# ruiguo-bio/smer_music_generation

Hardware: AMD Instinct MI355X
Metric: infill tokens/sec + train tokens/sec, SMER seq_len=1024, 1/2/4/8 MI355X (higher is better)
Workload: dtype bf16; 1 GPU; C2 train step: 6+6 layers d512 h8 ff2048 V309, per-GPU B=32 S=1024 T=256, dropout 0.1, fused WCE + Adam; global_batch=32, seq_len=1024, tgt_len=256, parallelism=dp1

## Files before the change

### include/smer_hip.h

```cpp
#ifndef SMER_HIP_H
#define SMER_HIP_H

#include <stddef.h>
#include <stdint.h>

#ifdef __cplusplus
extern "C" {
#endif

typedef struct ihipStream_t* smer_stream_t;

#define SMER_OK 0
#define SMER_ERR_INVALID (-1)
#define SMER_ERR_HIP (-2)
#define SMER_ERR_UNSUPPORTED (-3)

#define SMER_F32 0
#define SMER_BF16 1

int smer_abi_version(void);
const char* smer_last_error(void);

int smer_gemm(int dtype, int a_kcontig, int b_kcontig, int M, int N, int K,
              const void* A, long lda, const void* B, long ldb,
// ... 196 lines not shown
                         smer_stream_t stream);
int smer_bar_clock(int R, int V, float* logits, long ldl, const int32_t* state, int nst,
                   const int8_t* targets, int max_masks, const int32_t* out_tok, int cap,
                   const uint8_t* cls, const uint8_t* units, int eos, const int32_t* bar_len,
                   int32_t* clock, smer_stream_t stream);

int smer_layernorm_fwd(int dtype, int M, int N, const void* x, long ldx,
                       const float* gamma, const float* beta, float eps,
                       void* y, long ldy, float* mean, float* rstd, smer_stream_t stream);
size_t smer_layernorm_bwd_workspace(int M, int N);
int smer_layernorm_bwd(int dtype, int M, int N, const void* dy, long lddy, int dy_f32,
                       const void* x, long ldx, const float* mean, const float* rstd,
                       const float* gamma, void* dx, long lddx,
                       void* dx_drop, long ldxd, float drop_p, uint32_t seed,
                       float* dgamma, float* dbeta, int accumulate,
                       void* workspace, size_t ws_bytes, smer_stream_t stream);
int smer_layernorm_bwd_partials(int dtype, int M, int N, const void* dy, long lddy, int dy_f32,
                                const void* x, long ldx, const float* mean, const float* rstd,
                                const float* gamma, void* dx, long lddx, void* dx_drop,
                                long ldxd, float drop_p, uint32_t seed, void* workspace,
                                size_t ws_bytes, smer_stream_t stream);
int smer_layernorm_param_reduce(int M, int N, void* workspace, size_t ws_bytes, float* dgamma,
                                float* dbeta, int accumulate, smer_stream_t stream);

int smer_embed_fwd(int dtype, int n_tok, int d, const int64_t* ids, const int32_t* positions,
                   int L, const float* table, const float* pe, float scale,
                   float drop_p, uint32_t seed, void* out, long ldo, smer_stream_t stream);
int smer_embed_fwd_fp8(int n_tok, int d, const int64_t* ids, const int32_t* positions, int L,
                       const float* table, const float* pe, float scale, float drop_p, uint32_t seed,
                       void* out, long ldo, void* q8, long ldq, const float* qs, unsigned* amax,
                       smer_stream_t stream);
size_t smer_embed_bwd_workspace(int V, int d, int n_tok_total);
int smer_embed_bwd(int dtype, int V, int d, float scale,
                   const int64_t* ids0, const void* dx0, long ld0, int n0, float p0, uint32_t seed0,
                   const int64_t* ids1, const void* dx1, long ld1, int n1, float p1, uint32_t seed1,
                   float* dtable, void* workspace, size_t ws_bytes, smer_stream_t stream);

int smer_wce_denom(int n, const int64_t* y, const float* ce_all, float* denom,
                   smer_stream_t stream);
int smer_wce_fwd_bwd(int dtype, int R, int V, const float* logits, long ldl, const int64_t* y,
                     const float* w, const float* denom, float* row_loss, float* loss_out,
                     void* dlogits, long ldd, float grad_scale, smer_stream_t stream);

int smer_adam(long n, float* p, const float* g, float* m, float* v, void* p_bf16,
              float lr, float b1, float b2, float eps, float bc1, float bc2_sqrt,
              smer_stream_t stream);
// ... 59 lines not shown
```

### smer_music_generation_amd/_lib.py

```python
from __future__ import annotations

import ctypes
import os

import torch

_HERE = os.path.dirname(os.path.abspath(__file__))
LIB_PATH = os.environ.get("SMER_HIP_LIB") or os.path.join(_HERE, "libsmer_hip.so")

c_int, c_long, c_float, c_size, c_u32 = (ctypes.c_int, ctypes.c_long, ctypes.c_float,
                                         ctypes.c_size_t, ctypes.c_uint32)
P = ctypes.c_void_p

SIGNATURES = {
    "smer_abi_version": (c_int, []),
    "smer_last_error": (ctypes.c_char_p, []),
    "smer_gemm": (c_int, [c_int, c_int, c_int, c_int, c_int, c_int, P, c_long, P, c_long, P,
                          c_float, c_int, P, c_long, P, c_long, c_float, c_float, c_u32, P,
                          c_long, P, c_long, c_int, P, c_size, P]),
    "smer_gemm_debug_stamps": (c_int, [P, c_size]),
    "smer_gemm_plan": (c_int, [c_int, c_int, c_int, c_int, c_int, c_int, ctypes.c_uint, c_long, c_size, c_int,
                               c_int, P]),
    "smer_gemm_kernel_name": (ctypes.c_char_p, [c_int]),
    "smer_attn_fwd_plan": (c_int, [c_int, c_int, c_int, c_int, c_int, c_int, ctypes.c_uint, P]),
# ... 81 lines not shown
    "smer_grammar_sample_step": (c_int, [c_int, c_int, P, c_long, P, c_int, P, c_int, P, P, P,
                                         c_int, c_int, c_int, c_int, P, P, P, P, c_int, P, P, P,
                                         c_int, P]),
    "smer_grammar_sample_step_tp": (c_int, [c_int, c_int, P, c_long, P, c_int, P, c_int, P, P, P,
                                            c_int, c_int, c_int, c_int, P, P, P, P, c_int, P, P, P,
                                            c_int, P, P]),
    "smer_grammar_sample_step_rows": (c_int, [c_int, c_int, P, c_long, P, c_int, P, c_int, P, P, P,
                                              c_int, c_int, c_int, c_int, P, P, P, P, c_int, P, c_long,
                                              P, P, c_int, P, P]),
    "smer_logits_ban": (c_int, [c_int, c_int, P, c_long, P, c_int, c_int, P, P, c_int, P]),
    "smer_logprob_stage": (c_int, [c_int, c_int, P, c_long, P, c_int, P, c_int, P, P, c_long, P, P]),
    "smer_logprob_commit": (c_int, [c_int, c_int, P, c_int, P, P, c_int, P, c_long, P, P]),
    "smer_logprob_rows": (c_int, [c_int, c_int, c_int, P, c_long, P, P, P, P, P, c_int, P, P, P, P]),
    "smer_logits_template": (c_int, [c_int, c_int, P, c_long, P, c_int, P, P, c_int, c_int, P]),
    "smer_bar_clock": (c_int, [c_int, c_int, P, c_long, P, c_int, P, c_int, P, c_int, P, P, c_int, P, P, P]),
    "smer_layernorm_fwd": (c_int, [c_int, c_int, c_int, P, c_long, P, P, c_float, P, c_long, P,
                                   P, P]),
    "smer_layernorm_bwd_workspace": (c_size, [c_int, c_int]),
    "smer_layernorm_bwd": (c_int, [c_int, c_int, c_int, P, c_long, c_int, P, c_long, P, P, P, P,
                                   c_long, P, c_long, c_float, c_u32, P, P, c_int, P, c_size, P]),
    "smer_layernorm_bwd_partials": (c_int, [c_int, c_int, c_int, P, c_long, c_int, P, c_long, P, P,
                                            P, P, c_long, P, c_long, c_float, c_u32, P, c_size, P]),
    "smer_layernorm_param_reduce": (c_int, [c_int, c_int, P, c_size, P, P, c_int, P]),
    "smer_embed_fwd": (c_int, [c_int, c_int, c_int, P, P, c_int, P, P, c_float, c_float, c_u32,
                               P, c_long, P]),
    "smer_embed_bwd_workspace": (c_size, [c_int, c_int, c_int]),
    "smer_embed_bwd": (c_int, [c_int, c_int, c_int, c_float, P, P, c_long, c_int, c_float, c_u32,
                               P, P, c_long, c_int, c_float, c_u32, P, P, c_size, P]),
    "smer_wce_denom": (c_int, [c_int, P, P, P, P]),
    "smer_wce_fwd_bwd": (c_int, [c_int, c_int, c_int, P, c_long, P, P, P, P, P, P, c_long,
                                 c_float, P]),
    "smer_adam": (c_int, [c_long, P, P, P, P, P, c_float, c_float, c_float, c_float, c_float,
                          c_float, P]),
    "smer_cast": (c_int, [c_int, c_int, c_long, P, P, P]),
    "smer_cast2d": (c_int, [c_int, c_int, c_int, c_int, P, c_long, P, c_long, P]),
    "smer_colsum_workspace": (c_size, [c_int, c_int]),
    "smer_colsum": (c_int, [c_int, c_int, c_int, P, c_long, P, c_int, P, c_size, P]),
    "smer_debug_checksum": (c_int, [P, c_long, c_long, c_long, P, c_int, P]),
    "smer_argmax_accuracy": (c_int, [c_int, c_int, P, c_long, P, P, c_int, c_int, P, P]),
}

_lib = None
_load_error = None


def load():
# ... 29 lines not shown
```

### smer_music_generation_amd/csrc/common.h

```cpp
#pragma once
#include <hip/hip_runtime.h>
#include <stdint.h>

#include "../../include/smer_hip.h"

typedef __bf16 bf16;
typedef __bf16 bf16x8 __attribute__((ext_vector_type(8)));
typedef __bf16 bf16x4 __attribute__((ext_vector_type(4)));
typedef short i16x4 __attribute__((ext_vector_type(4)));
typedef float f32x4 __attribute__((ext_vector_type(4)));

#define SMER_WAVE 64

extern "C" int smer_set_error(int code, const char* msg);
#define SMER_CHECK_LAUNCH(what)                                          \
  do {                                                                   \
    hipError_t _e = hipGetLastError();                                   \
    if (_e != hipSuccess) return smer_set_error(SMER_ERR_HIP, hipGetErrorString(_e)); \
  } while (0)
#define SMER_REQUIRE(cond, msg) \
  do { if (!(cond)) return smer_set_error(SMER_ERR_INVALID, msg); } while (0)

template <typename T> __device__ __forceinline__ float to_f32(T x);
template <> __device__ __forceinline__ float to_f32<float>(float x) { return x; }
// ... 70 lines not shown
  h = __umul24(h, 0x6CA68Bu);
  h ^= h >> 16;
  return h;
}
__device__ __forceinline__ uint32_t smer_attn_ge(uint32_t h, uint32_t lo4) {
  return (h | 0x80808080u) - lo4;
}
__device__ __forceinline__ bool smer_attn_keep(uint32_t rowkey, uint32_t thr7, uint32_t key) {
  return ((smer_attn_bits(rowkey, key >> 2) >> (8 * (key & 3))) & 0x7Fu) >= thr7;
}
static inline uint32_t smer_attn_thr7(float p) {
  if (p <= 0.f) return 0u;
  long t = (long)((double)p * 128.0 + 0.5);
  return (uint32_t)(t < 1 ? 1 : (t > 127 ? 127 : t));
}
static inline float smer_attn_scale7(uint32_t thr7) {
  return thr7 ? (float)(128.0 / (128.0 - (double)thr7)) : 1.f;
}

size_t smer_col_reduce_scratch(int nblk, int N);
void smer_col_reduce_launch(int nblk, int N, const float* part, long stride, long off, float* out,
                            int accumulate, float scale, float* scratch, hipStream_t s,
                            float* out2 = nullptr, int nsplit = 0);

template <typename T, bool VEC = true>
__device__ __forceinline__ void load8(const T* p, int valid, float (&v)[8]) {
  if (VEC && valid >= 8) {
    if constexpr (sizeof(T) == 2) {
      bf16x8 r = *reinterpret_cast<const bf16x8*>(p);
#pragma unroll
      for (int i = 0; i < 8; ++i) v[i] = (float)r[i];
    } else {
      float4 a = *reinterpret_cast<const float4*>(p), b = *reinterpret_cast<const float4*>(p + 4);
      v[0] = a.x; v[1] = a.y; v[2] = a.z; v[3] = a.w; v[4] = b.x; v[5] = b.y; v[6] = b.z; v[7] = b.w;
    }
  } else {
#pragma unroll
    for (int i = 0; i < 8; ++i) v[i] = i < valid ? (float)p[i] : 0.f;
  }
}

constexpr int LNR_MAXC = 4;
template <int NC = LNR_MAXC>
__device__ __forceinline__ void ln_stats_loaded(const float (&v)[NC][8], int N, float eps, int lane, float& mu,
                                                float& rs) {
  const int nch = N >> 3;
// ... 168 lines not shown
```

### smer_music_generation_amd/csrc/norm_embed.hip

```cpp
#include "common.h"

namespace {
constexpr int LN_MAXC = 4;

template <typename T> struct Vec8;
template <> struct Vec8<bf16> {
  static __device__ __forceinline__ void load(const bf16* p, float (&v)[8]) {
    bf16x8 r = *reinterpret_cast<const bf16x8*>(p);
#pragma unroll
    for (int i = 0; i < 8; ++i) v[i] = (float)r[i];
  }
  static __device__ __forceinline__ void store(bf16* p, const float (&v)[8]) {
    bf16x8 r;
#pragma unroll
    for (int i = 0; i < 8; ++i) r[i] = (bf16)v[i];
    *reinterpret_cast<bf16x8*>(p) = r;
  }
};
template <> struct Vec8<float> {
  static __device__ __forceinline__ void load(const float* p, float (&v)[8]) {
    float4 a = *reinterpret_cast<const float4*>(p), b = *reinterpret_cast<const float4*>(p + 4);
    v[0] = a.x; v[1] = a.y; v[2] = a.z; v[3] = a.w; v[4] = b.x; v[5] = b.y; v[6] = b.z; v[7] = b.w;
  }
  static __device__ __forceinline__ void store(float* p, const float (&v)[8]) {
// ... 735 lines not shown
  if (!occ[which]) {
    int nb = 0;
    const void* kern = which == 2   ? (const void*)ln_bwd_t4_kernel<4>
                       : which == 0 ? (const void*)ln_bwd_kernel<bf16, false, 2, 2, true>
                                    : (const void*)ln_bwd_kernel<bf16, false, 4, 1, true>;
    if (hipOccupancyMaxActiveBlocksPerMultiprocessor(&nb, kern, 256, 0) != hipSuccess || nb <= 0) nb = 1;
    occ[which] = nb;
  }
  int dev = 0, cus = 256;
  if (hipGetDevice(&dev) != hipSuccess ||
      hipDeviceGetAttribute(&cus, hipDeviceAttributeMultiprocessorCount, dev) != hipSuccess || cus <= 0)
    cus = 256;
  const long resident = (long)cus * occ[which];
  const long per = (M + resident - 1) / resident;
  const int rows = (int)((per + 15) / 16 * 16);
  return rows > fixed ? fixed : rows;
}

extern "C" size_t smer_layernorm_bwd_workspace(int M, int N) {
  size_t nblk = (size_t)(M + ln_bwd_rows(M, N) - 1) / ln_bwd_rows(M, N);
  return nblk * 2 * N * sizeof(float) + smer_col_reduce_scratch((int)nblk, 2 * N);
}

static int ln_bwd_impl(int dtype, int M, int N, const void* dy, long lddy, int dy_f32,
                       const void* x, long ldx, const float* mean, const float* rstd,
                       const float* gamma, void* dx, long lddx, void* dx_drop, long ldxd,
                       float drop_p, uint32_t seed, float* dgamma, float* dbeta, int accumulate,
                       void* workspace, size_t ws_bytes, smer_stream_t stream, bool params,
                       bool reduce, uint8_t* q8 = nullptr, long ldq = 0, const float* qs = nullptr,
                       unsigned* amax = nullptr) {
  SMER_REQUIRE(N % 8 == 0 && N <= 64 * 8 * LN_MAXC, "smer_layernorm_bwd: N % 8 == 0 and N <= 2048");
  SMER_REQUIRE(dx && dy && x && mean && rstd && gamma, "smer_layernorm_bwd: null pointer");
  SMER_REQUIRE(!params || (workspace && ws_bytes >= smer_layernorm_bwd_workspace(M, N)),
               "smer_layernorm_bwd: workspace too small");
  if (M == 0) return SMER_OK;
  hipStream_t s = (hipStream_t)stream;
  const int rpb = ln_bwd_rows(M, N);
  int nblk = (M + rpb - 1) / rpb;
  uint32_t thr = smer_drop_thr16(drop_p);
  float ds = smer_drop_scale16(thr);
  float* part = params ? (float*)workspace : nullptr;
  SMER_REQUIRE(((uintptr_t)gamma & 15) == 0, "smer_layernorm_bwd: gamma must be 16-B aligned");
#define LNB2(T, F, NC, RB, PF)                                                                 \
  hipLaunchKernelGGL((ln_bwd_kernel<T, F, NC, RB, PF>), dim3(nblk), dim3(256), 0, s, M, N, dy, \
                     lddy, (const T*)x, ldx, mean, rstd, gamma, (T*)dx, lddx, (T*)dx_drop, ldxd, \
                     thr, seed, ds, part, rpb)
#define LNB1(T, F, NC, RB)                                          \
  do {                                                              \
    if (rpb / 4 > (RB)) LNB2(T, F, NC, RB, true);                   \
    else LNB2(T, F, NC, RB, false);                                 \
  } while (0)
#define LNB(T, F)                                  \
  do {                                             \
    if (N <= 512) LNB1(T, F, 1, 4);                \
    else if (N <= 1024) LNB1(T, F, 2, 2);          \
    else LNB1(T, F, 4, 1);                         \
// ... 99 lines not shown

extern "C" int smer_layernorm_param_reduce(int M, int N, void* workspace, size_t ws_bytes,
                                           float* dgamma, float* dbeta, int accumulate,
                                           smer_stream_t stream) {
  SMER_REQUIRE(workspace && ws_bytes >= smer_layernorm_bwd_workspace(M, N),
               "smer_layernorm_param_reduce: workspace too small");
  if (M == 0 || (!dgamma && !dbeta)) return SMER_OK;
  const int nblk = (M + ln_bwd_rows(M, N) - 1) / ln_bwd_rows(M, N);
  float* part = (float*)workspace;
  hipStream_t s = (hipStream_t)stream;
  if (dgamma && dbeta)
    smer_col_reduce_launch(nblk, 2 * N, part, (long)2 * N, 0L, dgamma, accumulate, 1.f,
                           part + (size_t)nblk * 2 * N, s, dbeta, N);
  else if (dgamma)
    smer_col_reduce_launch(nblk, N, part, (long)2 * N, 0L, dgamma, accumulate, 1.f,
                           part + (size_t)nblk * 2 * N, s);
  else
    smer_col_reduce_launch(nblk, N, part, (long)2 * N, (long)N, dbeta, accumulate, 1.f,
                           part + (size_t)nblk * 2 * N, s);
  SMER_CHECK_LAUNCH("smer_layernorm_param_reduce");
  return SMER_OK;
}

extern "C" int smer_embed_fwd(int dtype, int n_tok, int d, const int64_t* ids,
                              const int32_t* positions, int L, const float* table,
                              const float* pe, float scale, float drop_p, uint32_t seed,
                              void* out, long ldo, smer_stream_t stream) {
  SMER_REQUIRE(d % 4 == 0, "smer_embed_fwd: d % 4 == 0");
  SMER_REQUIRE(positions || L > 0, "smer_embed_fwd: L");
  if (n_tok == 0) return SMER_OK;
  hipStream_t s = (hipStream_t)stream;
  long tot = (long)n_tok * (d / 4);
  uint32_t thr = smer_drop_thr16(drop_p);
  float ds = smer_drop_scale16(thr);
  if (dtype == SMER_BF16)
    hipLaunchKernelGGL(embed_fwd_kernel<bf16>, dim3((tot + 255) / 256), dim3(256), 0, s, n_tok, d,
                       ids, positions, L, table, pe, scale, thr, seed, ds, (bf16*)out, ldo);
  else if (dtype == SMER_F32)
    hipLaunchKernelGGL(embed_fwd_kernel<float>, dim3((tot + 255) / 256), dim3(256), 0, s, n_tok, d,
                       ids, positions, L, table, pe, scale, thr, seed, ds, (float*)out, ldo);
  else
    return smer_set_error(SMER_ERR_UNSUPPORTED, "smer_embed_fwd: dtype");
  SMER_CHECK_LAUNCH("smer_embed_fwd");
  return SMER_OK;
}

// ... 59 lines not shown
```

### smer_music_generation_amd/csrc/train_ops.hip

```cpp
#include "common.h"

__global__ __launch_bounds__(256) void wce_denom_kernel(int n, const int64_t* __restrict__ y,
                                                        const float* __restrict__ ce_all,
                                                        float* __restrict__ denom) {
  __shared__ float red[256];
  float a = 0.f;
  for (int i = threadIdx.x; i < n; i += 256) a += ce_all[y[i]];
  red[threadIdx.x] = a;
  __syncthreads();
  for (int s = 128; s > 0; s >>= 1) {
    if (threadIdx.x < s) red[threadIdx.x] += red[threadIdx.x + s];
    __syncthreads();
  }
  if (threadIdx.x == 0) *denom = red[0];
}

template <typename T>
__global__ __launch_bounds__(256) void wce_kernel(int R, int V, const float* __restrict__ logits,
                                                  long ldl, const int64_t* __restrict__ y,
                                                  const float* __restrict__ w,
                                                  const float* __restrict__ denom,
                                                  float* __restrict__ row_loss,
                                                  T* __restrict__ dlog, long ldd,
                                                  float grad_scale) {
// ... 133 lines not shown

size_t smer_col_reduce_scratch(int nblk, int N) {
  return nblk > 64 ? (size_t)((nblk + 63) / 64) * N * sizeof(float) : 0;
}

void smer_col_reduce_launch(int nblk, int N, const float* part, long stride, long off, float* out,
                            int accumulate, float scale, float* scratch, hipStream_t s,
                            float* out2, int nsplit) {
  dim3 gx((N + 63) / 64);
  if (!out2) nsplit = N;
  if (nblk > 64) {
    int g = (nblk + 63) / 64;
    hipLaunchKernelGGL(smer_col_reduce, dim3(gx.x, g), dim3(256), 0, s, nblk, N, part, stride,
                       off, scratch, (long)N, 64, 0, 1.f, (float*)nullptr, N);
    hipLaunchKernelGGL(smer_col_reduce, dim3(gx.x, 1), dim3(256), 0, s, g, N,
                       (const float*)scratch, (long)N, 0L, out, 0L, g, accumulate, scale, out2,
                       nsplit);
  } else {
    hipLaunchKernelGGL(smer_col_reduce, dim3(gx.x, 1), dim3(256), 0, s, nblk, N, part, stride,
                       off, out, 0L, nblk, accumulate, scale, out2, nsplit);
  }
}

extern "C" int smer_wce_denom(int n, const int64_t* y, const float* ce_all, float* denom,
                              smer_stream_t stream) {
  SMER_REQUIRE(y && ce_all && denom, "smer_wce_denom: null pointer");
  hipLaunchKernelGGL(wce_denom_kernel, dim3(1), dim3(256), 0, (hipStream_t)stream, n, y, ce_all,
                     denom);
  SMER_CHECK_LAUNCH("smer_wce_denom");
  return SMER_OK;
}

extern "C" int smer_wce_fwd_bwd(int dtype, int R, int V, const float* logits, long ldl,
                                const int64_t* y, const float* w, const float* denom,
                                float* row_loss, float* loss_out, void* dlogits, long ldd,
                                float grad_scale, smer_stream_t stream) {
  SMER_REQUIRE(logits && y && w && denom && row_loss, "smer_wce_fwd_bwd: null pointer");
  if (R == 0) return SMER_OK;
  hipStream_t s = (hipStream_t)stream;
  dim3 grid((R + 3) / 4);
  if (dtype == SMER_BF16)
    hipLaunchKernelGGL(wce_kernel<bf16>, grid, dim3(256), 0, s, R, V, logits, ldl, y, w, denom,
                       row_loss, (bf16*)dlogits, ldd, grad_scale);
  else if (dtype == SMER_F32)
    hipLaunchKernelGGL(wce_kernel<float>, grid, dim3(256), 0, s, R, V, logits, ldl, y, w, denom,
                       row_loss, (float*)dlogits, ldd, grad_scale);
// ... 184 lines not shown
```

### smer_music_generation_amd/engine.py

```python
from __future__ import annotations

import math
import os

import torch

from . import ops

_SITE = {"pe_src": 1, "pe_tgt": 2}


def _site(kind, layer, which):
    return 16 + (layer * 16 + which) * 2 + (0 if kind == "enc" else 1)


class _W:
    pass


FP8_FFN2 = os.environ.get("SMER_FP8_FFN2", "1") == "1"
FP8_EMBED = os.environ.get("SMER_FP8_EMBED", "0") == "1"
FP8_H8 = (os.environ.get("SMER_FP8_H8", "1") == "1"
          and os.environ.get("SMER_FP8_Q8_FAST", "1") != "0")


_WGRAD_SIDE_CAP = int(os.environ.get("SMER_WGRAD_SIDE_CAP", "0"))
_WGRAD_FP8_CAP = int(os.environ.get("SMER_WGRAD_FP8_CAP", "192"))
_ATTN_MASK_PREGEN = os.environ.get("SMER_ATTN_MASK_PREGEN", "0") == "1"


class Engine:
    def __init__(self, model):
        self.m = model
        self.d = model.d_model
        self.H = model.nhead
        self.D = self.d // self.H
        self.F = model.dim_feedforward
        self.V = model.vocab_size
        self.Vp = (self.V + 63) // 64 * 64
        self.n_enc = model.num_encoder_layers
        self.n_dec = model.num_decoder_layers
        self._bf16 = None
        self._bf16_version = None
        self._fc_pad = None
        self._wgen = 0
        self._ckv_all = None
        self._side = {}
        self._mstream = {}
        self._fp8 = None

    def act_dtype(self):
        return torch.float32 if self.m.precision == "fp32" else torch.bfloat16

    def _weights_flat(self, dt):
        flat = self.m.flat_parameters()
        if dt == torch.float32:
            return flat
        ver = self._version_key()
        if self._bf16 is None or self._bf16.numel() != flat.numel() or self._bf16_version != ver:
            if self._bf16 is None or self._bf16.numel() != flat.numel():
                self._bf16 = torch.empty(flat.numel(), dtype=torch.bfloat16, device=flat.device)
            ops.cast(flat, self._bf16)
            self._fc_pad = None
            self._bf16_version = ver
            self._wgen += 1
        return self._bf16

    def _version_key(self):
        flat = self.m.flat_parameters()
        return (flat.data_ptr(), flat._version, sum(p._version for p in self.m.parameters()))

    def mark_bf16_fresh(self):
# ... 365 lines not shown
                return
            if x is None or dy is None:
                raise RuntimeError("engine: fp8 weight gradient declined with no bf16 input")
            ops.linear_wgrad(dy, x, gw, ws=ws, max_wg=cap, **kw)
        if side is None:
            run(None, 0)
            return
        stream, ws = side
        stream.wait_stream(torch.cuda.current_stream(side[1].device))
        with torch.cuda.stream(stream):
            run(ws, _WGRAD_SIDE_CAP)
            if ops.CK_LOG is not None:
                ops.ck("S:dW", gw)
                ops.ck("S:db", kw.get("db"))
                ops.ck("S:dy", dy)
                ops.ck("S:x", x)
        for t in (dy, x):
            if t is not None:
                t.record_stream(stream)
        if q8 is not None:
            q8[0].record_stream(stream)
            q8[2].record_stream(stream)

    @staticmethod
    def _join(side):
        if side is not None:
            torch.cuda.current_stream(side[0].device).wait_stream(side[0])

    @staticmethod
    def _hook(side, hook, name):
        if side is None:
            hook(name)
            return
        with torch.cuda.stream(side[0]):
            hook(name)

    def backward(self, ctx, dlog_pad, hook=None):
        m = self.m
        dt = ctx.dt
        dev = dlog_pad.device
        B, S, T = ctx.B, ctx.S, ctx.T
        d, H, D, V = self.d, self.H, self.D, self.V
        scale = 1.0 / math.sqrt(D)
        p_tr = ctx.p_tr
        sd = lambda site: (ctx.seed * 1000003 + site) & 0xFFFFFFFF
        W = self.weights(dt)
        G = self.grad_views()
        Mt, Ms = B * T, B * S

        from .fp8 import FP8_ATTN_DGRAD, FP8_DGRAD, eligible
        f8 = ctx.f8 if FP8_DGRAD else None

        def ln_bwd(g_in, y_, mu, rs, wb, dx_, dxd_, seed_, gw, site):
            kw = dict(dx_drop=dxd_ if p_tr > 0 else None, drop_p=p_tr, seed=seed_, dgamma=gw[0],
                      dbeta=gw[1], param_stream=ps)
            if f8 is None:
                ops.layernorm_bwd(g_in, y_, mu, rs, wb[0], dx_, **kw)
                if ops.CK_LOG is not None:
                    ops.ck("M:ln_in.g", g_in)
                    ops.ck("M:ln_in.y", y_)
                    ops.ck("M:ln_in.mu", mu)
                    ops.ck("M:ln_in.rs", rs)
                return None
            si = f8.site(site)
            q = torch.empty(y_.shape, dtype=torch.uint8, device=dev)
            ops.layernorm_bwd(g_in, y_, mu, rs, wb[0], dx_, q8=q, qs=f8.qs_of(si), amax=f8.amax_of(si), **kw)
            f8.record_bwd(site)
            return (q, si) if site in f8.bwd_ready else None

        def attn_q8(shape, site, parts):
            if f8 is None or not FP8_ATTN_DGRAD:
                return None, None
            si = f8.site(site)
            buf = torch.empty(shape, dtype=torch.uint8, device=dev)
            views = [None if p is None else buf[:, p[0]:p[1]] for p in parts]
            f8.record_bwd(site)
            return (views[0], views[1], views[2], f8.qs_of(si), f8.amax_of(si)), \
                ((buf, si) if site in f8.bwd_ready else None)
# ... 50 lines not shown
                raise RuntimeError("engine: %s e4m3-gated dgrad declined its shape" % name)
            f8.record_bwd(q_site)
            return out, ((q, si) if q_site in f8.bwd_ready else None)

        def q_only_grad(xq_, name, w, site, dropped=True):
            M = ctx.B * (ctx.S if name.startswith("enc") else ctx.T)
            return (FP8_H8 and (p_tr > 0 or not dropped) and f8 is not None and f8w is not None and xq_ is not None
                    and site in f8.bwd_ready and f8.weight_t(name) is not None
                    and eligible(M, w.shape[1], w.shape[0]) and w.shape[0] % 256 == 0 and M % 64 == 0)

        def dgrad_in(y_, xq_, name, w, site):
            if p_tr == 0:
                return None
            return None if q_only_grad(xq_, name, w, site) else torch.empty_like(y_)

        ops.ck("M:dlog", dlog_pad)
        wg(dlog_pad, ctx.dec_out, G.fc_w, M=V, db=G.fc_b)
        g_out = ops.linear_dgrad(dlog_pad, W.fc_pad, K=self.Vp)
        ck = ops.ck
        ck("M:g_out", g_out)
        y_last, mo, ro = ctx.dec_last
        dy = torch.empty_like(y_last)
        ops.layernorm_bwd(g_out, y_last, mo, ro, W.dec_norm[0], dy, dgamma=G.dec_norm[0],
                          dbeta=G.dec_norm[1], param_stream=ps)
        ck("M:dy_final", dy)
        if hook:
            self._hook(side, hook, "head")
        cross8 = None
        if f8 is not None and FP8_ATTN_DGRAD and self.n_dec:
            cross8 = (f8.site("b.cross"), torch.empty(Ms, self.n_dec * 2 * d, dtype=torch.uint8, device=dev))
        kv_q_only = (cross8 is not None and FP8_H8 and f8w is not None and "b.cross" in f8.bwd_ready
                     and ctx.memq is not None and f8.weight_t("ckv") is not None
                     and eligible(Ms, d, self.n_dec * 2 * d) and (2 * d) % 256 == 0 and Ms % 64 == 0)
        dkvc_all = None if kv_q_only else torch.empty(Ms, self.n_dec * 2 * d, dtype=dt, device=dev)
        for i in reversed(range(self.n_dec)):
            L, GL = W.dec[i], G.dec[i]
            (y_in, qkv, o, lse, y1, m1, r1, x1, qc, kvc, oc, lsec, y2, m2, r2, x2, h, y3, m3,
             r3) = ctx.dec[i]
            yq_in, oq, x1q, ocq, x2q, hq = ctx.dec_q[i]
            dy3 = torch.empty_like(y3)
            dy3d = dgrad_in(y3, hq, "dec%d.l2" % i, L.l2_w, "b.dec%d.ln3" % i) if p_tr > 0 else dy3
            dy3q = ln_bwd(dy, y3, m3, r3, L.n3, dy3, dy3d, sd(_site("dec", i, 5)), GL.n3, "b.dec%d.ln3" % i)
            ck("M:dec%d.dy3" % i, dy3d)
            dh, dhq = ffn2_bwd(dy3q, dy3d, "dec%d.l2" % i, L.l2_w, GL, h, hq, "b.dec%d.dh" % i, x2q,
                               "dec%d.l1" % i)
            ck("M:dec%d.dh" % i, dh)
            wg(dh, x2, GL.l1_w, dhq, x2q, db=GL.l1_b)
            dx2, _ = dgrad(dhq, dh, "dec%d.l1" % i, L.l1_w, residual=dy3)
            ck("M:dec%d.dx2" % i, dx2)
# ... 32 lines not shown
            ck("M:dec%d.dx1" % i, dx1)
            dy1 = torch.empty_like(y1)
            dy1d = dgrad_in(y1, oq, "dec%d.sao" % i, L.sa_ow, "b.dec%d.ln1" % i) if p_tr > 0 else dy1
            dy1q = ln_bwd(dx1, y1, m1, r1, L.n1, dy1, dy1d, sd(_site("dec", i, 1)), GL.n1, "b.dec%d.ln1" % i)
            ck("M:dec%d.dy1" % i, dy1d)
            wg(dy1d, o, GL.sa_ow, dy1q, oq, db=GL.sa_ob)
            do, _ = dgrad(dy1q, dy1d, "dec%d.sao" % i, L.sa_ow)
            ck("M:dec%d.do" % i, do)
            q8s, dqkvq = attn_q8((Mt, 3 * d), "b.dec%d.dqkv" % i, [(0, d), (d, 2 * d), (2 * d, 3 * d)])
            dqkv = None if (q8s is not None and q_only_grad(yq_in, "dec%d.sa" % i, L.sa_w, "b.dec%d.dqkv" % i,
                                                            dropped=False)) else \
                torch.empty(Mt, 3 * d, dtype=dt, device=dev)
            dq_, dk_, dv_ = (None, None, None) if dqkv is None else \
                (dqkv[:, :d], dqkv[:, d:2 * d], dqkv[:, 2 * d:])
            ops.attn_bwd(qkv[:, :d], qkv[:, d:2 * d], qkv[:, 2 * d:], o, do, lse, dq_,
                         dk_, dv_, B=B, H=H, Lq=T, Lk=T, D=D,
                         kpm=ctx.tkpm, causal=True, scale=scale, drop_p=p_tr,
                         seed=sd(_site("dec", i, 0)), drop_mask=ctx.masks.get(("dec", i)), q8=q8s)
            ck("M:dec%d.dqkv" % i, dqkv)
            wg(dqkv, y_in, GL.sa_w, dqkvq, yq_in, db=GL.sa_b)
            dy, _ = dgrad(dqkvq, dqkv, "dec%d.sa" % i, L.sa_w, residual=dy1)
            ck("M:dec%d.dy" % i, dy)
            if hook:
                self._hook(side, hook, "dec%d" % i)
        d_tgt = dy
        if self.n_dec:
            if kv_q_only or (cross8 is not None and "b.cross" in f8.bwd_ready and f8.weight_t("ckv") is not None
                             and eligible(Ms, d, self.n_dec * 2 * d)):
                dmem, _ = dgrad((cross8[1], cross8[0]), dkvc_all, "ckv", W.ckv_all)
            else:
                dmem = ops.linear_dgrad(dkvc_all, W.ckv_all, out_f32=torch.empty(Ms, d, device=dev))
        else:
            dmem = torch.zeros(Ms, d, device=dev)
        ck("M:dmem", dmem)
        x_last, me, re = ctx.enc_last
        dx = torch.empty_like(x_last)
        ops.layernorm_bwd(dmem, x_last, me, re, W.enc_norm[0], dx, dgamma=G.enc_norm[0],
                          dbeta=G.enc_norm[1], param_stream=ps)
        for i in reversed(range(self.n_enc)):
            L, GL = W.enc[i], G.enc[i]
            (x_in, qkv, o, lse, y1, m1, r1, x1, h, y2, m2, r2) = ctx.enc[i]
            xq_in, oq, x1q, hq = ctx.enc_q[i]
            dy2 = torch.empty_like(y2)
            dy2d = dgrad_in(y2, hq, "enc%d.l2" % i, L.l2_w, "b.enc%d.ln2" % i) if p_tr > 0 else dy2
            dy2q = ln_bwd(dx, y2, m2, r2, L.n2, dy2, dy2d, sd(_site("enc", i, 3)), GL.n2, "b.enc%d.ln2" % i)
            ck("M:enc%d.dy2" % i, dy2d)
            dh, dhq = ffn2_bwd(dy2q, dy2d, "enc%d.l2" % i, L.l2_w, GL, h, hq, "b.enc%d.dh" % i, x1q,
                               "enc%d.l1" % i)
            ck("M:enc%d.dh" % i, dh)
            wg(dh, x1, GL.l1_w, dhq, x1q, db=GL.l1_b)
            dx1, _ = dgrad(dhq, dh, "enc%d.l1" % i, L.l1_w, residual=dy2)
            ck("M:enc%d.dx1" % i, dx1)
            dy1 = torch.empty_like(y1)
            dy1d = dgrad_in(y1, oq, "enc%d.out" % i, L.out_w, "b.enc%d.ln1" % i) if p_tr > 0 else dy1
            dy1q = ln_bwd(dx1, y1, m1, r1, L.n1, dy1, dy1d, sd(_site("enc", i, 1)), GL.n1, "b.enc%d.ln1" % i)
            ck("M:enc%d.dy1" % i, dy1d)
            wg(dy1d, o, GL.out_w, dy1q, oq, db=GL.out_b)
            do, _ = dgrad(dy1q, dy1d, "enc%d.out" % i, L.out_w)
            ck("M:enc%d.do" % i, do)
            q8s, dqkvq = attn_q8((Ms, 3 * d), "b.enc%d.dqkv" % i, [(0, d), (d, 2 * d), (2 * d, 3 * d)])
            dqkv = None if (q8s is not None and q_only_grad(xq_in, "enc%d.in" % i, L.in_w, "b.enc%d.dqkv" % i,
                                                            dropped=False)) else \
                torch.empty(Ms, 3 * d, dtype=dt, device=dev)
            dq_, dk_, dv_ = (None, None, None) if dqkv is None else \
                (dqkv[:, :d], dqkv[:, d:2 * d], dqkv[:, 2 * d:])
            ops.attn_bwd(qkv[:, :d], qkv[:, d:2 * d], qkv[:, 2 * d:], o, do, lse, dq_,
                         dk_, dv_, B=B, H=H, Lq=S, Lk=S, D=D,
                         kpm=ctx.skpm, causal=False, scale=scale, drop_p=p_tr,
                         seed=sd(_site("enc", i, 0)), drop_mask=ctx.masks.get(("enc", i)), q8=q8s)
            ck("M:enc%d.dqkv" % i, dqkv)
            wg(dqkv, x_in, GL.in_w, dqkvq, xq_in, db=GL.in_b)
            dx, _ = dgrad(dqkvq, dqkv, "enc%d.in" % i, L.in_w, residual=dy1)
            ck("M:enc%d.dx" % i, dx)
            if hook:
                self._hook(side, hook, "enc%d" % i)
        ops.embed_bwd(G.emb, math.sqrt(d), [(ctx.src_ids, dx, ctx.p_pos, sd(_SITE["pe_src"])),
                                            (ctx.tgt_ids, d_tgt, ctx.p_pos, sd(_SITE["pe_tgt"]))])
        self._join(side)
        if hook:
            hook("embedding")


class ScoreTransformerFunction(torch.autograd.Function):
    @staticmethod
    def forward(fctx, anchor, model, need_grad, src, tgt, src_kpm, tgt_kpm, mem_kpm, tgt_mask):
        eng = model.engine
        if not src.is_cuda:
            raise RuntimeError("the SMER engine runs on the GPU: move the model and inputs to "
                               "a ROCm device first")
        training = model.training and (model.pos_dropout > 0 or model.trans_dropout > 0)
        seed = int(torch.randint(0, 2 ** 31 - 1, (1,)).item()) if training else 0
        logits, wts, ctx = eng.forward(src, tgt, src_kpm, tgt_kpm, mem_kpm,
                                       training=model.training, need_weights=model.need_weights,
                                       save=need_grad, seed=seed)
        fctx.eng = eng
        fctx.ctx = ctx
        fctx.model = model
        B, T = tgt.shape
# ... 17 lines not shown
```

### smer_music_generation_amd/ops.py

```python
from __future__ import annotations

import torch

from ._lib import call, load

F32, BF16 = 0, 1


def dtype_code(t: torch.dtype) -> int:
    if t == torch.float32:
        return F32
    if t == torch.bfloat16:
        return BF16
    raise TypeError("unsupported dtype %s" % t)


def _p(t):
    if t is None:
        return None
    if not t.is_cuda:
        raise RuntimeError("smer op: tensor must be on the GPU (got %s)" % t.device)
    return t.data_ptr()


# ... 699 lines not shown
                  (cls, torch.uint8), (units, torch.uint8), (bar_len, torch.int32), (clock, torch.int32)):
        if t.dtype != dt or t.device != logits.device:
            raise RuntimeError("bar_clock: expected %s on the logits' device" % dt)
    if not all(t.is_contiguous() for t in (state, targets, out_tok, cls, units, bar_len, clock)) or \
            logits.dim() != 2 or logits.stride(1) != 1:
        raise RuntimeError("bar_clock: expected contiguous tables and logits rows")
    if logits.shape[0] < 2 * R or targets.dim() != 2 or targets.shape[0] != R or targets.shape[1] < 1 or \
            out_tok.dim() != 2 or out_tok.shape[0] != R or out_tok.shape[1] < 1 or \
            tuple(cls.shape) != (V,) or tuple(units.shape) != (V,) or tuple(bar_len.shape) != (R,) or \
            tuple(clock.shape) != (R, CLOCK_WORDS) or not 1 <= V <= 512 or nst < 9:
        raise RuntimeError("bar_clock: shape mismatch")
    call("smer_bar_clock", R, V, _p(logits), _ld(logits), _p(state), nst, _p(targets), targets.shape[1],
         _p(out_tok), out_tok.shape[1], _p(cls), _p(units), int(eos), _p(bar_len), _p(clock), _stream())


def layernorm(x, gamma, beta, y, mean, rstd, eps=1e-5):
    M, N = x.shape
    call("smer_layernorm_fwd", dtype_code(x.dtype), M, N, _p(x), _ld(x), _p(gamma), _p(beta),
         float(eps), _p(y), _ld(y), _p(mean), _p(rstd), _stream())


def layernorm_bwd(dy, x, mean, rstd, gamma, dx, *, dx_drop=None, drop_p=0.0, seed=0,
                  dgamma=None, dbeta=None, accumulate=True, param_stream=None, q8=None, qs=None,
                  amax=None):
    lib = load()
    M, N = x.shape
    nbytes = lib.smer_layernorm_bwd_workspace(M, N) if (dgamma is not None or dbeta is not None) else 0
    ws = torch.empty(max(1, nbytes), dtype=torch.uint8, device=x.device)
    if q8 is not None:
        if x.dtype != torch.bfloat16 or dy.dtype != torch.bfloat16:
            raise RuntimeError("layernorm_bwd: the e4m3 copy needs bf16 dy and x")
        partial = param_stream is not None and nbytes > 0
        call("smer_layernorm_bwd_fp8", M, N, _p(dy), _ld(dy), _p(x), _ld(x), _p(mean), _p(rstd),
             _p(gamma), _p(dx), _ld(dx), _p(dx_drop), _ld(dx_drop) if dx_drop is not None else 0,
             float(drop_p), int(seed) & 0xFFFFFFFF, _p(q8), _ld(q8), _p(qs), _p(amax),
             _p(None if partial else dgamma), _p(None if partial else dbeta), int(accumulate),
             _p(ws), nbytes, int(partial), _stream())
        if partial:
            param_stream.wait_stream(torch.cuda.current_stream(x.device))
            with torch.cuda.stream(param_stream):
                call("smer_layernorm_param_reduce", M, N, _p(ws), nbytes, _p(dgamma), _p(dbeta),
                     int(accumulate), _stream())
            ws.record_stream(param_stream)
        return
    if param_stream is not None and nbytes:
        call("smer_layernorm_bwd_partials", dtype_code(x.dtype), M, N, _p(dy), _ld(dy),
             int(dy.dtype == torch.float32 and x.dtype != torch.float32), _p(x), _ld(x), _p(mean),
             _p(rstd), _p(gamma), _p(dx), _ld(dx), _p(dx_drop),
             _ld(dx_drop) if dx_drop is not None else 0, float(drop_p), int(seed) & 0xFFFFFFFF,
             _p(ws), nbytes, _stream())
        param_stream.wait_stream(torch.cuda.current_stream(x.device))
        with torch.cuda.stream(param_stream):
            call("smer_layernorm_param_reduce", M, N, _p(ws), nbytes, _p(dgamma), _p(dbeta),
                 int(accumulate), _stream())
        ws.record_stream(param_stream)
        return
    call("smer_layernorm_bwd", dtype_code(x.dtype), M, N, _p(dy), _ld(dy),
         int(dy.dtype == torch.float32 and x.dtype != torch.float32), _p(x), _ld(x), _p(mean),
         _p(rstd), _p(gamma), _p(dx), _ld(dx), _p(dx_drop),
         _ld(dx_drop) if dx_drop is not None else 0, float(drop_p), int(seed) & 0xFFFFFFFF,
         _p(dgamma), _p(dbeta), int(accumulate), _p(ws), nbytes, _stream())


def embed(ids, table, pe, out, *, L=0, positions=None, scale, drop_p=0.0, seed=0):
    n_tok = ids.numel()
    d = table.shape[1]
    call("smer_embed_fwd", dtype_code(out.dtype), n_tok, d, _p(ids), _p(positions), int(L),
         _p(table), _p(pe), float(scale), float(drop_p), int(seed) & 0xFFFFFFFF, _p(out),
         _ld(out), _stream())


def embed_fp8(ids, table, pe, out, q8, qs, amax, *, L=0, positions=None, scale, drop_p=0.0, seed=0):
    n_tok = ids.numel()
    d = table.shape[1]
    call("smer_embed_fwd_fp8", n_tok, d, _p(ids), _p(positions), int(L), _p(table), _p(pe), float(scale),
         float(drop_p), int(seed) & 0xFFFFFFFF, _p(out), _ld(out), _p(q8), _ld(q8), _p(qs), _p(amax), _stream())


def embed_bwd(dtable, scale, segs):
    lib = load()
    V, d = dtable.shape
    segs = list(segs) + [(None, None, 0.0, 0)] * (2 - len(segs))
    (i0, x0, p0, s0), (i1, x1, p1, s1) = segs
    n0 = i0.numel() if i0 is not None else 0
# ... 64 lines not shown
```

Measured before the change: 3.136 million train tokens/s (B*(S+T)).

## Batch LayerNorm parameter-gradient reductions into one multi-site kernel launch

LayerNorm backward now writes per-block dgamma/dbeta partials into slots of a preallocated persistent arena, and no longer launches a separate reduce per LN site on the side stream. One batched kernel then reduces all sites, driven by a device-side table, once per layer group at hook points or once at the end of backward. This removes per-site kernel launches, stream waits and per-call workspace allocations. In exchange the partials stay live in memory longer, and a new reduction kernel with a different summation order is added.

```diff
diff --git a/include/smer_hip.h b/include/smer_hip.h
--- a/include/smer_hip.h
+++ b/include/smer_hip.h
@@ -242,6 +242,15 @@
                                 size_t ws_bytes, smer_stream_t stream);
 int smer_layernorm_param_reduce(int M, int N, void* workspace, size_t ws_bytes, float* dgamma,
                                 float* dbeta, int accumulate, smer_stream_t stream);
+int smer_layernorm_bwd_nblk(int M, int N);
+typedef struct smer_ln_reduce_site {
+  const float* part;
+  float* dgamma;
+  float* dbeta;
+  int nblk, N, accumulate, reserved;
+} smer_ln_reduce_site;
+int smer_layernorm_param_reduce_batch(int nsites, const smer_ln_reduce_site* sites,
+                                      const smer_ln_reduce_site* sites_dev, smer_stream_t stream);
 
 int smer_embed_fwd(int dtype, int n_tok, int d, const int64_t* ids, const int32_t* positions,
                    int L, const float* table, const float* pe, float scale,
diff --git a/smer_music_generation_amd/_lib.py b/smer_music_generation_amd/_lib.py
--- a/smer_music_generation_amd/_lib.py
+++ b/smer_music_generation_amd/_lib.py
@@ -127,6 +127,8 @@
     "smer_layernorm_bwd_partials": (c_int, [c_int, c_int, c_int, P, c_long, c_int, P, c_long, P, P,
                                             P, P, c_long, P, c_long, c_float, c_u32, P, c_size, P]),
     "smer_layernorm_param_reduce": (c_int, [c_int, c_int, P, c_size, P, P, c_int, P]),
+    "smer_layernorm_bwd_nblk": (c_int, [c_int, c_int]),
+    "smer_layernorm_param_reduce_batch": (c_int, [c_int, P, P, P]),
     "smer_embed_fwd": (c_int, [c_int, c_int, c_int, P, P, c_int, P, P, c_float, c_float, c_u32,
                                P, c_long, P]),
     "smer_embed_bwd_workspace": (c_size, [c_int, c_int, c_int]),
diff --git a/smer_music_generation_amd/csrc/common.h b/smer_music_generation_amd/csrc/common.h
--- a/smer_music_generation_amd/csrc/common.h
+++ b/smer_music_generation_amd/csrc/common.h
@@ -116,6 +116,9 @@
 void smer_col_reduce_launch(int nblk, int N, const float* part, long stride, long off, float* out,
                             int accumulate, float scale, float* scratch, hipStream_t s,
                             float* out2 = nullptr, int nsplit = 0);
+constexpr int SMER_LN_REDUCE_MAX_NBLK = 64 * 64;
+void smer_ln_param_reduce_batch_launch(int nsites, int max_cols, const smer_ln_reduce_site* sites_dev,
+                                       hipStream_t s);
 
 template <typename T, bool VEC = true>
 __device__ __forceinline__ void load8(const T* p, int valid, float (&v)[8]) {
diff --git a/smer_music_generation_amd/csrc/norm_embed.hip b/smer_music_generation_amd/csrc/norm_embed.hip
--- a/smer_music_generation_amd/csrc/norm_embed.hip
+++ b/smer_music_generation_amd/csrc/norm_embed.hip
@@ -781,6 +781,12 @@
   return nblk * 2 * N * sizeof(float) + smer_col_reduce_scratch((int)nblk, 2 * N);
 }
 
+extern "C" int smer_layernorm_bwd_nblk(int M, int N) {
+  if (M <= 0 || N <= 0) return 0;
+  const int rpb = ln_bwd_rows(M, N);
+  return (M + rpb - 1) / rpb;
+}
+
 static int ln_bwd_impl(int dtype, int M, int N, const void* dy, long lddy, int dy_f32,
                        const void* x, long ldx, const float* mean, const float* rstd,
                        const float* gamma, void* dx, long lddx, void* dx_drop, long ldxd,
@@ -790,7 +796,9 @@
                        unsigned* amax = nullptr) {
   SMER_REQUIRE(N % 8 == 0 && N <= 64 * 8 * LN_MAXC, "smer_layernorm_bwd: N % 8 == 0 and N <= 2048");
   SMER_REQUIRE(dx && dy && x && mean && rstd && gamma, "smer_layernorm_bwd: null pointer");
-  SMER_REQUIRE(!params || (workspace && ws_bytes >= smer_layernorm_bwd_workspace(M, N)),
+  SMER_REQUIRE(!params || (workspace && ws_bytes >= (reduce ? smer_layernorm_bwd_workspace(M, N)
+                                                            : (size_t)smer_layernorm_bwd_nblk(M, N) * 2 * N *
+                                                                  sizeof(float))),
                "smer_layernorm_bwd: workspace too small");
   if (M == 0) return SMER_OK;
   hipStream_t s = (hipStream_t)stream;
@@ -936,6 +944,26 @@
   return SMER_OK;
 }
 
+extern "C" int smer_layernorm_param_reduce_batch(int nsites, const smer_ln_reduce_site* sites,
+                                                 const smer_ln_reduce_site* sites_dev,
+                                                 smer_stream_t stream) {
+  if (nsites == 0) return SMER_OK;
+  SMER_REQUIRE(nsites > 0 && nsites <= 65535 && sites && sites_dev,
+               "smer_layernorm_param_reduce_batch: 1..65535 sites, host and device table");
+  int max_cols = 0;
+  for (int i = 0; i < nsites; ++i) {
+    const smer_ln_reduce_site& t = sites[i];
+    SMER_REQUIRE(t.part && (t.dgamma || t.dbeta), "smer_layernorm_param_reduce_batch: null pointer in a site");
+    SMER_REQUIRE(t.nblk >= 1 && t.nblk <= SMER_LN_REDUCE_MAX_NBLK && t.N >= 1 && t.N <= 64 * 8 * LN_MAXC,
+                 "smer_layernorm_param_reduce_batch: 1 <= nblk <= 4096 and 1 <= N <= 2048 per site");
+    const int cols = (t.dgamma && t.dbeta) ? 2 * t.N : t.N;
+    if (cols > max_cols) max_cols = cols;
+  }
+  smer_ln_param_reduce_batch_launch(nsites, max_cols, sites_dev, (hipStream_t)stream);
+  SMER_CHECK_LAUNCH("smer_layernorm_param_reduce_batch");
+  return SMER_OK;
+}
+
 extern "C" int smer_embed_fwd(int dtype, int n_tok, int d, const int64_t* ids,
                               const int32_t* positions, int L, const float* table,
                               const float* pe, float scale, float drop_p, uint32_t seed,
diff --git a/smer_music_generation_amd/csrc/train_ops.hip b/smer_music_generation_amd/csrc/train_ops.hip
--- a/smer_music_generation_amd/csrc/train_ops.hip
+++ b/smer_music_generation_amd/csrc/train_ops.hip
@@ -179,6 +179,95 @@
   }
 }
 
+__device__ __forceinline__ float col_reduce_group(const float* p, long stride, int b0, int b1, int g) {
+  float a0 = 0.f, a1 = 0.f, a2 = 0.f, a3 = 0.f;
+  int b = b0 + g;
+  for (; b + 12 < b1; b += 16) {
+    a0 += p[(long)b * stride];
+    a1 += p[(long)(b + 4) * stride];
+    a2 += p[(long)(b + 8) * stride];
+    a3 += p[(long)(b + 12) * stride];
+  }
+  for (; b < b1; b += 4) a0 += p[(long)b * stride];
+  return (a0 + a1) + (a2 + a3);
+}
+
+__global__ void __launch_bounds__(256) smer_ln_param_reduce_batch(const smer_ln_reduce_site* __restrict__ sites) {
+  __shared__ float red[2][4][64];
+  __shared__ float csum[SMER_LN_REDUCE_MAX_NBLK / 64][64];
+  const smer_ln_reduce_site st = sites[blockIdx.y];
+  const int cl = threadIdx.x & 63, g = threadIdx.x >> 6;
+  const int nblk = st.nblk, N = st.N;
+  const bool both = st.dgamma && st.dbeta;
+  const int ncol = both ? 2 * N : N;
+  if ((int)blockIdx.x * 64 >= ncol || (!st.dgamma && !st.dbeta) || nblk <= 0 ||
+      nblk > SMER_LN_REDUCE_MAX_NBLK)
+    return;
+  const long stride = 2L * N;
+  const int col = blockIdx.x * 64 + cl;
+  const bool live = col < ncol;
+  const float* p = st.part + (st.dgamma ? 0 : N) + (live ? col : 0);
+  float* out = st.dgamma ? st.dgamma : st.dbeta;
+  const int nsplit = both ? N : ncol;
+  float total;
+  if (nblk <= 64) {
+    red[0][g][cl] = live ? col_reduce_group(p, stride, 0, nblk, g) : 0.f;
+    __syncthreads();
+    total = (red[0][0][cl] + red[0][1][cl]) + (red[0][2][cl] + red[0][3][cl]);
+  } else {
+    const int nch = (nblk + 63) / 64, nfull = nblk / 64;
+    float v[16];
+#pragma unroll
+    for (int i = 0; i < 16; ++i) v[i] = live ? p[(long)(g + 4 * i) * stride] : 0.f;
+    for (int c = 0; c < nfull; ++c) {
+      float w[16];
+      if (c + 1 < nfull) {
+#pragma unroll
+        for (int i = 0; i < 16; ++i) w[i] = live ? p[(long)((c + 1) * 64 + g + 4 * i) * stride] : 0.f;
+      }
+      float a0 = 0.f, a1 = 0.f, a2 = 0.f, a3 = 0.f;
+#pragma unroll
+      for (int k = 0; k < 4; ++k) {
+        a0 += v[4 * k];
+        a1 += v[4 * k + 1];
+        a2 += v[4 * k + 2];
+        a3 += v[4 * k + 3];
+      }
+      red[c & 1][g][cl] = (a0 + a1) + (a2 + a3);
+      __syncthreads();
+      if (g == 0)
+        csum[c][cl] = (red[c & 1][0][cl] + red[c & 1][1][cl]) + (red[c & 1][2][cl] + red[c & 1][3][cl]);
+      if (c + 1 < nfull) {
+#pragma unroll
+        for (int i = 0; i < 16; ++i) v[i] = w[i];
+      }
+    }
+    if (nch > nfull) {
+      const int c = nfull;
+      red[c & 1][g][cl] = live ? col_reduce_group(p, stride, c * 64, nblk, g) : 0.f;
+      __syncthreads();
+      if (g == 0)
+        csum[c][cl] = (red[c & 1][0][cl] + red[c & 1][1][cl]) + (red[c & 1][2][cl] + red[c & 1][3][cl]);
+    }
+    __syncthreads();
+    const float r = col_reduce_group(&csum[0][cl], 64, 0, nch, g);
+    red[0][g][cl] = r;
+    __syncthreads();
+    total = (red[0][0][cl] + red[0][1][cl]) + (red[0][2][cl] + red[0][3][cl]);
+  }
+  if (g == 0 && live) {
+    float* o = col < nsplit ? out + col : st.dbeta + (col - nsplit);
+    *o = st.accumulate ? *o + total : total;
+  }
+}
+
+void smer_ln_param_reduce_batch_launch(int nsites, int max_cols, const smer_ln_reduce_site* sites_dev,
+                                       hipStream_t s) {
+  if (nsites <= 0 || max_cols <= 0) return;
+  hipLaunchKernelGGL(smer_ln_param_reduce_batch, dim3((max_cols + 63) / 64, nsites), dim3(256), 0, s,
+                     sites_dev);
+}
+
 extern "C" int smer_wce_denom(int n, const int64_t* y, const float* ce_all, float* denom,
                               smer_stream_t stream) {
   SMER_REQUIRE(y && ce_all && denom, "smer_wce_denom: null pointer");
diff --git a/smer_music_generation_amd/engine.py b/smer_music_generation_amd/engine.py
--- a/smer_music_generation_amd/engine.py
+++ b/smer_music_generation_amd/engine.py
@@ -27,6 +27,11 @@
 _WGRAD_SIDE_CAP = int(os.environ.get("SMER_WGRAD_SIDE_CAP", "0"))
 _WGRAD_FP8_CAP = int(os.environ.get("SMER_WGRAD_FP8_CAP", "192"))
 _ATTN_MASK_PREGEN = os.environ.get("SMER_ATTN_MASK_PREGEN", "0") == "1"
+_LN_PARAM_BATCH = os.environ.get("SMER_LN_PARAM_BATCH", "1") != "0"
+
+
+class _LnParamPlan:
+    pass
 
 
 class Engine:
@@ -48,6 +53,7 @@
         self._side = {}
         self._mstream = {}
         self._fp8 = None
+        self._ln_plan = {}
 
     def act_dtype(self):
         return torch.float32 if self.m.precision == "fp32" else torch.bfloat16
@@ -459,6 +465,36 @@
             q8[0].record_stream(stream)
             q8[2].record_stream(stream)
 
+    def _ln_param_plan(self, dev, Mt, Ms, G):
+        key = (Mt, Ms, self.m.flat_grad().data_ptr())
+        plan = self._ln_plan.get(dev)
+        if plan is not None and plan.key == key:
+            return plan
+        d = self.d
+        sites = [("head", "dec_norm", Mt, G.dec_norm)]
+        for i in reversed(range(self.n_dec)):
+            sites += [("dec%d" % i, "dec%d.n%d" % (i, k), Mt, getattr(G.dec[i], "n%d" % k)) for k in (3, 2, 1)]
+        sites.append(("enc%d" % (self.n_enc - 1) if self.n_enc else "tail", "enc_norm", Ms, G.enc_norm))
+        for i in reversed(range(self.n_enc)):
+            sites += [("enc%d" % i, "enc%d.n%d" % (i, k), Ms, getattr(G.enc[i], "n%d" % k)) for k in (2, 1)]
+        sites = [s for s in sites if 0 < ops.ln_bwd_partial_bytes(s[2], d) <= ops.LN_REDUCE_MAX_NBLK * 2 * d * 4]
+        sizes = [(ops.ln_bwd_partial_bytes(M, d) + 255) // 256 * 256 for _, _, M, _ in sites]
+        plan = _LnParamPlan()
+        plan.key = key
+        plan.arena = torch.empty(max(1, sum(sizes)), dtype=torch.uint8, device=dev)
+        plan.slots, rows, off = {}, [], 0
+        for (group, name, M, gw), n in zip(sites, sizes):
+            plan.slots[name] = plan.arena[off:off + n]
+            rows.append((group, (plan.slots[name], M, d, gw[0], gw[1], True)))
+            off += n
+        plan.groups = {}
+        for group, _ in rows:
+            if group not in plan.groups:
+                plan.groups[group] = ops.LnReduceTable([r for g_, r in rows if g_ == group], dev)
+        plan.all = ops.LnReduceTable([r for _, r in rows], dev)
+        self._ln_plan[dev] = plan
+        return plan
+
     @staticmethod
     def _join(side):
         if side is not None:
@@ -488,9 +524,35 @@
         from .fp8 import FP8_ATTN_DGRAD, FP8_DGRAD, eligible
         f8 = ctx.f8 if FP8_DGRAD else None
 
+        lnp = self._ln_param_plan(dev, Mt, Ms, G) if _LN_PARAM_BATCH else None
+        ln_slot = (lambda name: lnp.slots.get(name)) if lnp is not None else (lambda name: None)
+        ln_flushed = set()
+
+        def ln_flush(group=None):
+            if lnp is None:
+                return
+            if group is not None:
+                tabs = [lnp.groups[group]] if group in lnp.groups and group not in ln_flushed else []
+                ln_flushed.add(group)
+            elif not ln_flushed:
+                tabs = [lnp.all]
+            else:
+                tabs = [t for g_, t in lnp.groups.items() if g_ not in ln_flushed]
+            tabs = [t for t in tabs if t.n]
+            if not tabs:
+                return
+            if ps is None:
+                for t in tabs:
+                    ops.ln_param_reduce_batch(t)
+                return
+            ps.wait_stream(torch.cuda.current_stream(dev))
+            with torch.cuda.stream(ps):
+                for t in tabs:
+                    ops.ln_param_reduce_batch(t)
+
         def ln_bwd(g_in, y_, mu, rs, wb, dx_, dxd_, seed_, gw, site):
             kw = dict(dx_drop=dxd_ if p_tr > 0 else None, drop_p=p_tr, seed=seed_, dgamma=gw[0],
-                      dbeta=gw[1], param_stream=ps)
+                      dbeta=gw[1], param_stream=ps, param_slot=ln_slot(site[2:].replace(".ln", ".n")))
             if f8 is None:
                 ops.layernorm_bwd(g_in, y_, mu, rs, wb[0], dx_, **kw)
                 if ops.CK_LOG is not None:
@@ -587,9 +649,10 @@
         y_last, mo, ro = ctx.dec_last
         dy = torch.empty_like(y_last)
         ops.layernorm_bwd(g_out, y_last, mo, ro, W.dec_norm[0], dy, dgamma=G.dec_norm[0],
-                          dbeta=G.dec_norm[1], param_stream=ps)
+                          dbeta=G.dec_norm[1], param_stream=ps, param_slot=ln_slot("dec_norm"))
         ck("M:dy_final", dy)
         if hook:
+            ln_flush("head")
             self._hook(side, hook, "head")
         cross8 = None
         if f8 is not None and FP8_ATTN_DGRAD and self.n_dec:
@@ -668,6 +731,7 @@
             dy, _ = dgrad(dqkvq, dqkv, "dec%d.sa" % i, L.sa_w, residual=dy1)
             ck("M:dec%d.dy" % i, dy)
             if hook:
+                ln_flush("dec%d" % i)
                 self._hook(side, hook, "dec%d" % i)
         d_tgt = dy
         if self.n_dec:
@@ -682,7 +746,7 @@
         x_last, me, re = ctx.enc_last
         dx = torch.empty_like(x_last)
         ops.layernorm_bwd(dmem, x_last, me, re, W.enc_norm[0], dx, dgamma=G.enc_norm[0],
-                          dbeta=G.enc_norm[1], param_stream=ps)
+                          dbeta=G.enc_norm[1], param_stream=ps, param_slot=ln_slot("enc_norm"))
         for i in reversed(range(self.n_enc)):
             L, GL = W.enc[i], G.enc[i]
             (x_in, qkv, o, lse, y1, m1, r1, x1, h, y2, m2, r2) = ctx.enc[i]
@@ -719,7 +783,9 @@
             dx, _ = dgrad(dqkvq, dqkv, "enc%d.in" % i, L.in_w, residual=dy1)
             ck("M:enc%d.dx" % i, dx)
             if hook:
+                ln_flush("enc%d" % i)
                 self._hook(side, hook, "enc%d" % i)
+        ln_flush()
         ops.embed_bwd(G.emb, math.sqrt(d), [(ctx.src_ids, dx, ctx.p_pos, sd(_SITE["pe_src"])),
                                             (ctx.tgt_ids, d_tgt, ctx.p_pos, sd(_SITE["pe_tgt"]))])
         self._join(side)
diff --git a/smer_music_generation_amd/ops.py b/smer_music_generation_amd/ops.py
--- a/smer_music_generation_amd/ops.py
+++ b/smer_music_generation_amd/ops.py
@@ -745,33 +745,41 @@
 
 def layernorm_bwd(dy, x, mean, rstd, gamma, dx, *, dx_drop=None, drop_p=0.0, seed=0,
                   dgamma=None, dbeta=None, accumulate=True, param_stream=None, q8=None, qs=None,
-                  amax=None):
+                  amax=None, param_slot=None):
     lib = load()
     M, N = x.shape
-    nbytes = lib.smer_layernorm_bwd_workspace(M, N) if (dgamma is not None or dbeta is not None) else 0
-    ws = torch.empty(max(1, nbytes), dtype=torch.uint8, device=x.device)
+    if param_slot is not None:
+        nbytes = ln_bwd_partial_bytes(M, N)
+        if param_slot.dtype != torch.uint8 or not param_slot.is_contiguous() or param_slot.numel() < nbytes:
+            raise RuntimeError("layernorm_bwd: param_slot must be contiguous uint8 of >= %d bytes" % nbytes)
+        ws, param_stream = param_slot, None
+    else:
+        nbytes = lib.smer_layernorm_bwd_workspace(M, N) if (dgamma is not None or dbeta is not None) else 0
+        ws = torch.empty(max(1, nbytes), dtype=torch.uint8, device=x.device)
     if q8 is not None:
         if x.dtype != torch.bfloat16 or dy.dtype != torch.bfloat16:
             raise RuntimeError("layernorm_bwd: the e4m3 copy needs bf16 dy and x")
-        partial = param_stream is not None and nbytes > 0
+        partial = (param_stream is not None or param_slot is not None) and nbytes > 0
         call("smer_layernorm_bwd_fp8", M, N, _p(dy), _ld(dy), _p(x), _ld(x), _p(mean), _p(rstd),
              _p(gamma), _p(dx), _ld(dx), _p(dx_drop), _ld(dx_drop) if dx_drop is not None else 0,
              float(drop_p), int(seed) & 0xFFFFFFFF, _p(q8), _ld(q8), _p(qs), _p(amax),
              _p(None if partial else dgamma), _p(None if partial else dbeta), int(accumulate),
              _p(ws), nbytes, int(partial), _stream())
-        if partial:
+        if partial and param_slot is None:
             param_stream.wait_stream(torch.cuda.current_stream(x.device))
             with torch.cuda.stream(param_stream):
                 call("smer_layernorm_param_reduce", M, N, _p(ws), nbytes, _p(dgamma), _p(dbeta),
                      int(accumulate), _stream())
             ws.record_stream(param_stream)
         return
-    if param_stream is not None and nbytes:
+    if (param_stream is not None or param_slot is not None) and nbytes:
         call("smer_layernorm_bwd_partials", dtype_code(x.dtype), M, N, _p(dy), _ld(dy),
              int(dy.dtype == torch.float32 and x.dtype != torch.float32), _p(x), _ld(x), _p(mean),
              _p(rstd), _p(gamma), _p(dx), _ld(dx), _p(dx_drop),
              _ld(dx_drop) if dx_drop is not None else 0, float(drop_p), int(seed) & 0xFFFFFFFF,
              _p(ws), nbytes, _stream())
+        if param_slot is not None:
+            return
         param_stream.wait_stream(torch.cuda.current_stream(x.device))
         with torch.cuda.stream(param_stream):
             call("smer_layernorm_param_reduce", M, N, _p(ws), nbytes, _p(dgamma), _p(dbeta),
@@ -783,6 +791,39 @@
          _p(rstd), _p(gamma), _p(dx), _ld(dx), _p(dx_drop),
          _ld(dx_drop) if dx_drop is not None else 0, float(drop_p), int(seed) & 0xFFFFFFFF,
          _p(dgamma), _p(dbeta), int(accumulate), _p(ws), nbytes, _stream())
+
+
+LN_REDUCE_MAX_NBLK = 4096
+
+
+def ln_bwd_partial_bytes(M, N):
+    return load().smer_layernorm_bwd_nblk(M, N) * 2 * N * 4
+
+
+class LnReduceTable:
+
+    def __init__(self, sites, device):
+        import numpy as np
+        dt = np.dtype([("part", "<u8"), ("dgamma", "<u8"), ("dbeta", "<u8"), ("nblk", "<i4"), ("N", "<i4"),
+                       ("accumulate", "<i4"), ("reserved", "<i4")])
+        lib = load()
+        host = np.zeros(len(sites), dtype=dt)
+        for i, (slot, M, N, dgamma, dbeta, accumulate) in enumerate(sites):
+            nblk = lib.smer_layernorm_bwd_nblk(M, N)
+            if slot.dtype != torch.uint8 or not slot.is_contiguous() or slot.numel() < nblk * 2 * N * 4:
+                raise RuntimeError("LnReduceTable: slot %d too small for [%d][%d] partials" % (i, nblk, 2 * N))
+            for t in (dgamma, dbeta):
+                if t is not None and (t.dtype != torch.float32 or not t.is_contiguous() or t.numel() != N):
+                    raise RuntimeError("LnReduceTable: dgamma / dbeta must be contiguous float32 [N]")
+            host[i] = (_p(slot), _p(dgamma) or 0, _p(dbeta) or 0, nblk, N, int(bool(accumulate)), 0)
+        self.host = host
+        self.dev = torch.from_numpy(host.view(np.uint8).copy()).to(device) if len(sites) else None
+        self.n = len(sites)
+
+
+def ln_param_reduce_batch(table):
+    if table.n:
+        call("smer_layernorm_param_reduce_batch", table.n, table.host.ctypes.data, _p(table.dev), _stream())
 
 
 def embed(ids, table, pe, out, *, L=0, positions=None, scale, drop_p=0.0, seed=0):
```

Measured after the change: 3.188 million train tokens/s (B*(S+T)), median of 6. 1.02x the previous value.
